# alibaba-mmai-research/CLIP-FSAR

Measured on AMD Instinct MI355X. Metric: episodes/sec (5-way 1-shot, 8 frames, ViT-B/16), higher is better.
Workload: dtype bf16; 1 GPU; BASELINE config[1]: 5-way 1-shot, 1 query/class, 8x224^2 frames, ViT-B/16, random-init CLIP weights, synthetic structured frames; frames_per_episode=80, precision=bf16, parallelism=episodes sharded over 1 rank(s); one all-gather of accuracies, launcher=single process

## Files before the change

clip-fsar_amd/build.py:

```python
from __future__ import annotations

import collections
import os
import subprocess
import sys

HERE = os.path.dirname(os.path.abspath(__file__))
CSRC = os.path.join(HERE, "csrc")
LIB = os.path.join(HERE, "libclipfsar_hip.so")
SOURCES = ["runtime.hip", "gemm.hip", "gemm_vit.hip", "frame_gemm.hip", "rowops.hip", "attention.hip", "tail.hip", "conv.hip"]
HIPCC = os.environ.get("HIPCC", "/opt/rocm/bin/hipcc")
DEV_LIB = os.path.join(HERE, "libclipfsar_hip_dev.so")
FLAGS = ["--offload-arch=gfx950", "-O3", "-std=c++17", "-fPIC", "-fvisibility=hidden", "-Wall", "-Wno-unused-function",
         "-Rpass-analysis=kernel-resource-usage"]
NO_PACKED_FP32 = ["-Xclang", "-target-feature", "-Xclang", "-packed-fp32-ops"]
SOURCE_FLAGS = {src: NO_PACKED_FP32 for src in SOURCES}
USAGE = os.path.join(HERE, "build", "resource_usage.json")
SideLib = collections.namedtuple("SideLib", "source lib usage")
SIDE_LIBS = {name: SideLib(name + ".hip", os.path.join(HERE, "libclipfsar_%s.so" % name),
                           os.path.join(HERE, "build", name, "resource_usage.json"))
             for name in ("gallery", "gallery_text", "stream", "pool", "ingest", "live")}


MORE_SIDE_LIBS = {name: SideLib(name + ".hip", os.path.join(HERE, "libclipfsar_%s.so" % name),
                                os.path.join(HERE, "build", name, "resource_usage.json"))
                  for name in ("groups",)}


def side_lib_names() -> list:
    return list(SIDE_LIBS)


def every_side_lib_names() -> list:
    return list(SIDE_LIBS) + list(MORE_SIDE_LIBS)


def _side_lib(name) -> SideLib:
    return SIDE_LIBS[name] if name in SIDE_LIBS else MORE_SIDE_LIBS[name]


def _parse_usage(text: str) -> dict:
    import re
    out, cur = {}, None
    for line in text.splitlines():
        m = re.search(r"remark: Function Name: (\S+)", line)
        if m:
            cur = out.setdefault(m.group(1), {})
            continue
        if cur is None:
            continue
        for key, pat in (("vgprs", r"remark:\s+VGPRs: (\d+)"), ("agprs", r"remark:\s+AGPRs: (\d+)"),
                         ("scratch", r"ScratchSize \[bytes/lane\]: (\d+)"), ("spills", r"VGPRs Spill: (\d+)"),
                         ("occupancy", r"Occupancy \[waves/SIMD\]: (\d+)")):
            m = re.search(pat, line)
            if m:
                cur[key] = int(m.group(1))
    return out


def _includes(path, seen=None) -> set:
    import re
    seen = set() if seen is None else seen
    path = os.path.normpath(path)
    if path not in seen:
        seen.add(path)
        for inc in re.findall(r'^#include "([^"]+)"', open(path).read(), flags=re.M):
            _includes(os.path.join(os.path.dirname(path), inc), seen)
    return seen


def _side_deps(name) -> list:
    return sorted(_includes(os.path.join(CSRC, _side_lib(name).source))) + [os.path.abspath(__file__)]


def _product_deps() -> list:
    ours = set().union(*(_includes(os.path.join(CSRC, s)) for s in SOURCES))
    side_only = set().union(*(_includes(os.path.join(CSRC, sl.source)) for sl in map(_side_lib, every_side_lib_names()))) - ours
    return [p for p in (os.path.join(CSRC, f) for f in sorted(os.listdir(CSRC))) if p not in side_only] + [
        os.path.join(os.path.dirname(HERE), "include", "clipfsar_hip.h"), os.path.abspath(__file__)]


def _stale(lib, deps) -> bool:
    if not os.path.exists(lib):
        return True
    t = os.path.getmtime(lib)
    return any(os.path.getmtime(d) > t for d in deps)


PACKED_LIB = os.path.join(HERE, "libclipfsar_hip_packed.so")


def _compile(src, obj, extra, verbose) -> dict:
    cmd = [HIPCC] + FLAGS + extra + ["-c", os.path.join(CSRC, src), "-o", obj]
    if verbose:
        print(" ".join(cmd), flush=True)
    p = subprocess.run(cmd, stdout=subprocess.PIPE, stderr=subprocess.STDOUT, text=True)
    if p.returncode != 0:
        raise RuntimeError("hipcc failed on %s:\n%s" % (src, p.stdout))
    rest = "\n".join(l for l in p.stdout.splitlines() if "-Rpass-analysis=kernel-resource-usage" not in l)
    if verbose and rest.strip():
        print(rest)
    return _parse_usage(p.stdout)


def _link(lib, objs, usage, usage_path, verbose) -> str:
    import json
    with open(usage_path, "w") as f:
        json.dump(usage, f, indent=0, sort_keys=True)
    cmd = [HIPCC, "--offload-arch=gfx950", "-shared", "-fPIC", "-o", lib] + objs
    if verbose:
        print(" ".join(cmd), flush=True)
    subprocess.check_call(cmd)
    return lib


def build_side(name, force: bool = False, verbose: bool = True) -> str:
    sl = _side_lib(name)
    if not force and not _stale(sl.lib, _side_deps(name)):
        return sl.lib
    bdir = os.path.dirname(sl.usage)
    os.makedirs(bdir, exist_ok=True)
    obj = os.path.join(bdir, sl.source.replace(".hip", ".o"))
    return _link(sl.lib, [obj], _compile(sl.source, obj, NO_PACKED_FP32, verbose), sl.usage, verbose)


def build(force: bool = False, verbose: bool = True, dev: bool = False, packed: bool = False, variant: str = "", defs=()) -> str:
    if not (dev or packed or variant):
        for name in every_side_lib_names():
            build_side(name, force=force, verbose=verbose)
    LIB_OUT = os.path.join(HERE, "libclipfsar_hip_%s.so" % variant) if variant else (PACKED_LIB if packed else (DEV_LIB if dev else LIB))
    if not force and not _stale(LIB_OUT, _product_deps()):
        return LIB_OUT
    bdir = os.path.join(HERE, "build", variant or "packed") if (packed or variant) else (os.path.join(HERE, "build", "dev") if dev else os.path.join(HERE, "build"))
    os.makedirs(bdir, exist_ok=True)
    extra = (os.environ.get("CFSAR_BUILD_DEFS", "").split() if dev else []) + list(defs)
    fenced = not (packed or "-DCFSAR_PACKED_FP32" in extra)
    extra = (["-DCFSAR_DEV"] if dev else []) + [e for e in extra if e != "-DCFSAR_PACKED_FP32"]
    objs = [os.path.join(bdir, src.replace(".hip", ".o")) for src in SOURCES]
    from concurrent.futures import ThreadPoolExecutor
    with ThreadPoolExecutor(len(SOURCES)) as pool:
        reports = list(pool.map(lambda so: _compile(so[0], so[1], extra + (SOURCE_FLAGS.get(so[0], []) if fenced else []), verbose),
                                zip(SOURCES, objs)))
    usage = {}
    for r in reports:
        usage.update(r)
    return _link(LIB_OUT, objs, usage, USAGE if not (dev or packed or variant) else os.path.join(bdir, "resource_usage.json"), verbose)


if __name__ == "__main__":
    _v = sys.argv[sys.argv.index("--variant") + 1] if "--variant" in sys.argv else ""
    _d = [a for a in sys.argv[1:] if a.startswith("-D")]
    print(build(force="--force" in sys.argv, dev="--dev" in sys.argv, packed="--packed" in sys.argv, variant=_v, defs=_d))
```

clip-fsar_amd/engine.py:

```python
from __future__ import annotations

import math

import os

import torch

from . import hip


FP16_SPLIT_DEFAULT = ""
FP16_MCORR_DEFAULT = "qkv,out,fc,pr"
FP16_STRICT_SPLIT_DEFAULT = "qkv"
FP16_STRICT_MCORR_DEFAULT = "out,fc,pr"
FP16_STRICT_DEEP_LAYERS = 12
FP16_STRICT_SPLIT_DEEP_DEFAULT = "qkv,fc"
FP16_STRICT_MCORR_DEEP_DEFAULT = "out,pr"


def _round_up(x, m):
    return (x + m - 1) // m * m


class HipViT:

    OPTIONS = {"fp16_wide": True, "fp16_lo": True, "fp16_rawmeans": True, "fused_umeans": True, "fused_omeans": True, "fuse_stats": True,
               "fused_patch": True, "strict_front": True, "strict_o_pair": False}

    def __init__(self, arch: dict, sd: dict, prefix: str = "", precision: str = "bf16", device="cuda", stream_dtype=None, fp16_split=None, fp16_mcorr=None,
                 options=None):
        self.strict = precision == "fp16_strict"
        if self.strict:
            precision = "fp16"
        if precision not in ("bf16", "fp16", "fp32"):
            raise ValueError("precision must be 'bf16', 'fp16', 'fp16_strict' or 'fp32'")
        opt = dict(self.OPTIONS)
        for k, v in (options or {}).items():
            if k not in opt:
                raise ValueError("HipViT: unknown option %r (known: %s)" % (k, ", ".join(sorted(opt))))
            opt[k] = bool(v)
        self.arch = dict(arch)
        self.precision = precision
        self.dev = torch.device(device)
        self.cd = {"bf16": torch.bfloat16, "fp16": torch.float16, "fp32": torch.float32}[precision]
        if stream_dtype is None:
            stream_dtype = "fp32" if precision == "fp32" else "fp16"
        if stream_dtype not in ("fp16", "fp32") or (precision == "fp32" and stream_dtype != "fp32") or (precision == "fp16" and stream_dtype != "fp16"):
            raise ValueError("stream_dtype must be 'fp32' (bf16 / fp32 precision) or 'fp16' (bf16 / fp16 precision)")
        self.xd = torch.float16 if stream_dtype == "fp16" else torch.float32
        D, P = arch["width"], arch["patch"]
        if D != arch["heads"] * 64:
            raise ValueError("HipViT needs head_dim == 64 (width %d, heads %d)" % (D, arch["heads"]))
        self.D, self.P, self.L, self.H, self.E = D, P, arch["layers"], arch["heads"], arch["embed"]
        self.grid = arch["res"] // P
        self.ntok = self.grid * self.grid + 1
        kq = 32 if precision == "fp32" else 64
        self.kpad = _round_up(3 * P * P, kq)

        def g(name):
            t = sd[prefix + name]
            if not isinstance(t, torch.Tensor):
                t = torch.from_numpy(t)
            return t.detach().to(device=self.dev, dtype=torch.float32).contiguous()

        cd = self.cd
        wc = torch.zeros(D, self.kpad, device=self.dev, dtype=torch.float32)
        wc[:, :3 * P * P] = g("conv1.weight").reshape(D, -1)
        self.w_patch = wc.to(cd).contiguous()
        self.fused_patch = bool(opt["fused_patch"] and P in hip.PATCH_EMBED_SLOTS and cd in (torch.bfloat16, torch.float16)
                                and self.xd == torch.float16)
        if self.fused_patch:
            self.w_patch_fused = self.w_patch if P == 16 else hip.patch_embed_weight(g("conv1.weight"), P, cd)
        self.cls = g("class_embedding")
        self.pos = g("positional_embedding")
        self.ln_pre = (g("ln_pre.weight"), g("ln_pre.bias"))
        self.ln_post = (g("ln_post.weight"), g("ln_post.bias"))
        self.w_proj_t = g("proj").t().contiguous()
        self.blocks = []
        for i in range(self.L):
            b = "transformer.resblocks.%d." % i
            self.blocks.append(dict(
                ln1=(g(b + "ln_1.weight"), g(b + "ln_1.bias")),
                ln2=(g(b + "ln_2.weight"), g(b + "ln_2.bias")),
                w_qkv=g(b + "attn.in_proj_weight").to(cd).contiguous(), b_qkv=g(b + "attn.in_proj_bias"),
                w_out=g(b + "attn.out_proj.weight").to(cd).contiguous(), b_out=g(b + "attn.out_proj.bias"),
                w_fc=g(b + "mlp.c_fc.weight").to(cd).contiguous(), b_fc=g(b + "mlp.c_fc.bias"),
                w_pr=g(b + "mlp.c_proj.weight").to(cd).contiguous(), b_pr=g(b + "mlp.c_proj.bias")))
        self.fold = (precision in ("bf16", "fp16") and self.xd == torch.float16 and D % 64 == 0 and D >= 128
                     and (precision == "fp16" or os.environ.get("CFSAR_LN_FOLD", "1") != "0"))
        if precision == "fp16":
            if not self.fold:
                raise ValueError("precision 'fp16' needs the LayerNorm-folded block (width a multiple of 64, >= 128)")
            wmax16 = max(float(blk[k].float().abs().max()) for blk in self.blocks for k in ("w_out", "w_pr"))
            wmax16 = max(wmax16, float(self.w_patch.float().abs().max()))
            if not wmax16 < 6.0e4:
                raise ValueError("precision 'fp16': a weight exceeds the fp16 range (max |w| = %.3g); use 'bf16' or 'fp32'" % wmax16)
        self.wide = precision == "fp16" and opt["fp16_wide"]
        self.two_word = self.wide and opt["fp16_lo"]
        sp_default, mc_default = FP16_SPLIT_DEFAULT, FP16_MCORR_DEFAULT
        if self.strict:
            deep = self.L > FP16_STRICT_DEEP_LAYERS
            sp_default = FP16_STRICT_SPLIT_DEEP_DEFAULT if deep else FP16_STRICT_SPLIT_DEFAULT
            mc_default = FP16_STRICT_MCORR_DEEP_DEFAULT if deep else FP16_STRICT_MCORR_DEFAULT
        sp = os.environ.get("CFSAR_FP16_SPLIT", sp_default if fp16_split is None else fp16_split) if precision == "fp16" else ""
        self.split = set(t for t in sp.split(",") if t)
        mc = os.environ.get("CFSAR_FP16_MCORR", mc_default if fp16_mcorr is None else fp16_mcorr) if precision == "fp16" else ""
        self.mcorr = set(t for t in mc.split(",") if t)
        if not (self.split | self.mcorr) <= {"qkv", "out", "fc", "pr"}:
            raise ValueError("CFSAR_FP16_SPLIT / CFSAR_FP16_MCORR: names out of qkv,out,fc,pr expected, got %r / %r" % (sp, mc))
        self.mcorr -= self.split
        if self.mcorr and self.ntok < 128:
            self.split |= self.mcorr
            self.mcorr = set()
        if not self.wide and precision == "fp16" and (self.mcorr or self.split & {"out", "pr"}):
            import warnings
            warnings.warn("HipViT: option fp16_wide=False drops the per-frame correction / split residual weights (%s / %s)" % (
                ",".join(sorted(self.mcorr)) or "-", ",".join(sorted(self.split & {"out", "pr"})) or "-"))
            self.mcorr = set()
            self.split -= {"out", "pr"}

        def hilo(W32):
            hi = W32.to(torch.float16)
            lo = (W32 - hi.float()).to(torch.float16)
            return torch.cat([hi, lo], 1).contiguous()

        def lo_word(W32):
            return (W32 - W32.to(torch.float16).float()).to(torch.bfloat16).contiguous()

        last = len(self.blocks) - 1
        for i, blk in enumerate(self.blocks if (self.split or self.mcorr) else []):
            b = "transformer.resblocks.%d." % i
            for key, name in (("out", "attn.out_proj.weight"), ("pr", "mlp.c_proj.weight")):
                if key in self.split:
                    blk["w_" + key] = hilo(g(b + name))
                elif key in self.mcorr:
                    blk["wlo_" + key] = lo_word(g(b + name))
                    if i == last:
                        blk["ws_" + key] = hilo(g(b + name))
        if self.fold:
            for i, blk in enumerate(self.blocks):
                b = "transformer.resblocks.%d." % i
                for tag, wname, bname, ln in (("qkv", "attn.in_proj_weight", "attn.in_proj_bias", "ln1"),
                                              ("fc", "mlp.c_fc.weight", "mlp.c_fc.bias", "ln2")):
                    W = g(b + wname)
                    gamma, beta = blk[ln]
                    if tag in self.split:
                        Wg = hilo(W * gamma[None, :])
                    else:
                        Wg = (W * gamma[None, :]).to(torch.float16).contiguous()
                    if tag in self.mcorr:
                        blk["wlo_" + tag] = lo_word(W * gamma[None, :])
                        if i == len(self.blocks) - 1:
                            Ws = hilo(W * gamma[None, :]) if tag == "fc" else hilo((W * gamma[None, :])[:D])
                            blk["wgs_" + tag] = Ws
                            blk["cs_" + tag] = Ws.double().sum(1).float().contiguous()
                    blk["wg_" + tag] = Wg
                    blk["c_" + tag] = Wg.double().sum(1).float().contiguous()
                    blk["cx_" + tag] = (W * gamma[None, :]).double().sum(1).float().contiguous()
                    blk["d_" + tag] = (W.double() @ beta.double() + g(b + bname).double()).float().contiguous()
            big = max(float(max(blk[k].abs().max() for k in ("c_qkv", "d_qkv", "c_fc", "d_fc"))) for blk in self.blocks)
            wmax = max(float(max(blk[k].float().abs().max() for k in ("wg_qkv", "wg_fc"))) for blk in self.blocks)
            if not (big < 3.0e4 and wmax < 6.0e4):
                import warnings
                if precision == "fp16":
                    raise ValueError("precision 'fp16': folded weights / vectors exceed the fp16 range (max |c|,|d| = %.3g, "
                                     "max |W gamma| = %.3g); use 'bf16' or 'fp32'" % (big, wmax))
                warnings.warn("LayerNorm folding disabled: folded weights / vectors exceed the fp16 range (max |c|,|d| = %.3g, "
                              "max |W gamma| = %.3g); using the unfolded block" % (big, wmax))
                self.fold = False
            if self.fold:
                for blk in self.blocks:
                    blk["w_qkv"] = blk["w_fc"] = None
        self.prune_last = os.environ.get("CFSAR_FULL_LAST_BLOCK", "0") != "1"
        self.fuse_stats = bool(self.fold) and hip.lnfold_partials_ok(self.D, self.D // 64) and opt["fuse_stats"]
        self.fused_umeans = opt["fused_umeans"]
        self.fused_omeans = opt["fused_omeans"]
        self.rawmeans = (opt["fp16_rawmeans"] and self.fused_umeans and self.fused_omeans
                         and all(k in self.mcorr for k in ("out", "pr")) and all(k in self.mcorr | self.split for k in ("qkv", "fc"))
                         and bool(self.mcorr & {"qkv", "fc"}))
        if self.rawmeans:
            for i, blk in enumerate(self.blocks):
                bb = "transformer.resblocks.%d." % i
                blk["wb_out"] = g(bb + "attn.out_proj.weight").to(torch.bfloat16).contiguous()
                blk["wb_pr"] = g(bb + "mlp.c_proj.weight").to(torch.bfloat16).contiguous()
        if self.mcorr & {"qkv", "fc"}:
            self.fuse_stats = False
        self.strict_front = self.o_pair = False
        if self.strict:
            if not (self.two_word and self.fold and D % 4 == 0 and D <= 1024):
                raise ValueError("precision 'fp16_strict' needs the two-word stream (options fp16_wide / fp16_lo) and a width <= 1024")
            self.strict_front = bool(opt["strict_front"])
            if self.strict_front:
                self.fused_patch = False
                w32 = wc
                w_hi = w32.to(torch.float16)
                w_lo = (w32 - w_hi.float()).to(torch.float16)
                self.w_patch3 = torch.cat([w_hi, w_hi, w_lo], 1).contiguous()
            self.o_pair = bool(opt["strict_o_pair"]) and self.fused_omeans and "out" in self.mcorr and D % 128 == 0
            if self.o_pair:
                for i, blk in enumerate(self.blocks):
                    W = g("transformer.resblocks.%d.attn.out_proj.weight" % i)
                    Wh = W.to(torch.float16)
                    blk["w3_out"] = torch.cat([Wh, Wh, (W - Wh.float()).to(torch.float16)], 1).contiguous()
        self._slots = {}
        self.max_frames_32bit = (2 ** 32 - 1) // (self.ntok * 4 * self.D * 2) - 1
        if self.strict_front:
            self.max_frames_32bit = min(self.max_frames_32bit, (2 ** 32 - 1) // ((self.ntok - 1) * 3 * self.kpad * 2) - 1)

    def _workspace(self, F_, slot=0):
        cap, ws = self._slots.get(slot, (0, None))
        if F_ > cap:
            M, D, cd, dev = F_ * self.ntok, self.D, self.cd, self.dev
            ws = dict(
                x=torch.empty(M, D, device=dev, dtype=self.xd),
                h=torch.empty(M, D, device=dev, dtype=cd),
                qkv=torch.empty(M, 3 * D, device=dev, dtype=cd),
                o=torch.empty(M, 2 * D if self.o_pair else D, device=dev, dtype=cd),
                u=torch.empty(M, 4 * D, device=dev, dtype=cd),
                c=torch.empty(F_, D, device=dev, dtype=torch.float32))
            if self.strict_front:
                ws["patches"] = torch.empty(F_ * (self.ntok - 1), 3 * self.kpad, device=dev, dtype=cd)
                ws["tok32"] = torch.empty(F_ * (self.ntok - 1), D, device=dev, dtype=torch.float32)
            elif not self.fused_patch:
                ws["patches"] = torch.empty(F_ * (self.ntok - 1), self.kpad, device=dev, dtype=cd)
            if self.fold:
                ws["part"] = torch.empty(M, D // 64, 2, device=dev, dtype=torch.float32)
                ws["rstat"] = torch.empty(M, 4, device=dev, dtype=torch.float32)
            if self.mcorr:
                ws["colsum"] = torch.empty((M // 96 + 2) * 2 * 4 * D, device=dev, dtype=torch.int32)
                ws["mU"] = torch.empty(F_ * 4 * D, device=dev, dtype=torch.bfloat16)
                ws["mX"] = torch.empty(F_, D, device=dev, dtype=torch.bfloat16)
                ws["xbar"] = torch.empty(F_, D, device=dev, dtype=torch.bfloat16)
                ws["mA"] = torch.empty(F_ * 4 * D, device=dev, dtype=torch.bfloat16)
                ws["corr"] = torch.empty(F_ * 4 * D, device=dev, dtype=torch.float32)
            if self.two_word:
                ws["xlo"] = torch.empty(M, D, device=dev, dtype=torch.float16)
                ws["xlc"] = torch.empty(F_, D, device=dev, dtype=torch.float16)
                ws["c32"] = torch.empty(F_, D, device=dev, dtype=torch.float32)
            ws["xc"] = torch.empty(F_, D, device=dev, dtype=self.xd)
            ws["hc"] = torch.empty(F_, D, device=dev, dtype=cd)
            ws["oc"] = torch.empty(F_, D, device=dev, dtype=cd)
            ws["uc"] = torch.empty(F_, 4 * D, device=dev, dtype=cd)
            ws["partc"] = torch.empty(F_, D // 64 if D % 64 == 0 else 1, 2, device=dev, dtype=torch.float32)
            ws["rstatc"] = torch.empty(F_, 4, device=dev, dtype=torch.float32)
            self._slots[slot] = (F_, ws)
        return ws

    def forward(self, frame_sets, feats_out=None, row_maps=None, taps=None, slot=0):
        if isinstance(frame_sets, torch.Tensor):
            frame_sets = [frame_sets]
        counts = [int(f.shape[0]) for f in frame_sets]
        F_ = sum(counts)
        if row_maps is None:
            row_maps, off = [], 0
            for c in counts:
                row_maps.append((0, 0, off))
                off += c
        if feats_out is None:
            feats_out = torch.empty(F_, self.E, device=self.dev, dtype=torch.float32)
        ws = self._workspace(F_, slot)
        N, D, npatch = self.ntok, self.D, self.ntok - 1
        M = F_ * N
        x, h, qkv, o, u = ws["x"], ws["h"], ws["qkv"], ws["o"], ws["u"]
        off = 0
        for fr, c in zip(frame_sets, counts):
            if fr.shape[1:] != (3, self.arch["res"], self.arch["res"]):
                raise RuntimeError("frames must be [F,3,%d,%d], got %s" % (self.arch["res"], self.arch["res"], tuple(fr.shape)))
            if self.fused_patch:
                hip.patch_embed(fr, self.w_patch_fused, self.pos, self.cls, x[off * N:(off + c) * N], self.P)
            elif self.strict_front:
                hip.im2col_patches_split(fr, ws["patches"][off * npatch:(off + c) * npatch], self.P)
            else:
                hip.im2col_patches(fr, ws["patches"][off * npatch:(off + c) * npatch], self.P)
            off += c
        if self.strict_front:
            hip.gemm(ws["patches"], self.w_patch3, ws["tok32"], M=F_ * npatch, N=D, K=3 * self.kpad, ldo=D)
            hip.embed_finish_pair(ws["tok32"], self.cls, self.pos, self.ln_pre[0], self.ln_pre[1], x, ws["xlo"], F_, N, D)
        else:
            if not self.fused_patch:
                hip.gemm(ws["patches"], self.w_patch, x, residual=self.pos, M=F_ * npatch, N=D, K=self.kpad, ldo=D, ldr=D,
                         row_group=npatch, row_gap=1, row_off=1, res_mod=npatch, res_off=1)
                hip.cls_rows(x, self.cls, self.pos, F_, N, D)
            hip.layernorm(x, x, self.ln_pre[0], self.ln_pre[1], M, D)
        if taps is not None:
            taps["ln_pre"] = (x[:M].float() + ws["xlo"][:M].float()) if self.strict_front else x[:M].clone()
        xc_final = None
        es = x.element_size()

        def class_rows(src, dst, row_elems, elem_bytes):
            hip.copy_rows_strided(src, N * row_elems * elem_bytes, dst, row_elems * elem_bytes, F_, row_elems * elem_bytes)

        if self.fold:
            part, rstat, S = ws["part"], ws["rstat"], D // 64
            xlo = ws["xlo"] if self.two_word else None
            if xlo is not None and not self.strict_front:
                xlo[:M].zero_()
            hip.row_stats(x, rstat, M, D)
            prune = self.prune_last and taps is None
            fuse = self.fuse_stats
            in_part = False
            split = self.split

            mcorr = self.mcorr
            raw = self.rawmeans and bool(mcorr)
            xbar = ws["xbar"][:F_] if raw else None
            if raw:
                hip.frame_col_means(x, xbar, F_, N)

            def mc(blk, key, A, rs=None, wrows=None, means=None):
                if key not in mcorr:
                    return None
                wlo = blk["wlo_" + key] if wrows is None else blk["wlo_" + key][wrows]
                Kd, Nn = A.shape[1], wlo.shape[0]
                if raw and key in ("qkv", "fc"):
                    mA = xbar
                elif means is not None:
                    mA = means
                else:
                    mA = ws["mA"][:F_ * Kd].view(F_, Kd)
                    hip.frame_col_means(A, mA, F_, N, rowstats=rs)
                cr = ws["corr"][:F_ * Nn].view(F_, Nn)
                hip.corr_gemm(mA, wlo, cr)
                return cr

            def fold(xx, wg, out, c, d, pt, rs, act=hip.ACT_NONE, rows=M, from_part=False, sp=False, corr=None, umeans=None, corr_raw=False):
                if sp or corr is not None or umeans is not None:
                    hip.gemm_lnfold_hp(xx, wg, out, c, d, rowstats=None if from_part else rs, partial=pt if from_part else None,
                                       slots=S if from_part else 0, rowstats_ws=rs, act=act, M=rows, wsplit=sp, corr=corr,
                                       corr_tokens=N if (corr is not None or umeans is not None) else 0, colmean_out=umeans,
                                       colsum_ws=ws["colsum"] if umeans is not None else None, corr_raw=corr_raw and corr is not None)
                elif from_part:
                    hip.gemm_lnfold_partials(xx, wg, out, c, d, pt, S, rs, act=act, M=rows)
                else:
                    hip.gemm_lnfold(xx, wg, out, c, d, rs, act=act, M=rows)

            def resid(A, blk, key, xx, xl, pt, rows, corr=None, cls=False):
                if self.o_pair and key == "out" and not cls:
                    hip.gemm_residual_wide(A, blk["w3_out"], xx, xl, blk["b_out"], pt, M=rows, wsplit=2)
                elif self.wide and cls and key in mcorr:
                    hip.gemm_residual_wide(A, blk["ws_" + key], xx, xl, blk["b_" + key], pt, M=rows, wsplit=True)
                elif self.wide:
                    hip.gemm_residual_wide(A, blk["w_" + key], xx, xl, blk["b_" + key], pt, M=rows, wsplit=key in split, corr=corr,
                                           corr_tokens=N if corr is not None else 0)
                else:
                    hip.gemm_residual_stats(A, blk["w_" + key], xx, blk["b_" + key], pt, M=rows)

            for i, b in enumerate(self.blocks):
                if prune and i == self.L - 1:
                    xc, oc, uc, partc, rstatc = ws["xc"][:F_], ws["oc"][:F_], ws["uc"][:F_], ws["partc"][:F_], ws["rstatc"][:F_]
                    xlc = ws["xlc"][:F_] if xlo is not None else None
                    kv = qkv.view(-1)[:M * 2 * D].view(M, 2 * D)
                    fold(x, b["wg_qkv"][D:], kv, b["cx_qkv" if raw else "c_qkv"][D:], b["d_qkv"][D:], part, rstat, from_part=in_part, sp="qkv" in split,
                         corr=mc(b, "qkv", x, rstat, wrows=slice(D, 3 * D)), corr_raw=raw)
                    class_rows(x, xc, D, es)
                    if xlo is not None:
                        class_rows(xlo, xlc, D, 2)
                    if in_part:
                        class_rows(part, partc, 2 * S, 4)
                    else:
                        class_rows(rstat, rstatc, 4, 4)
                    qc = ws["hc"][:F_]
                    if "qkv" in mcorr:
                        fold(xc, b["wgs_qkv"], qc, b["cs_qkv"], b["d_qkv"][:D], partc, rstatc, rows=F_, from_part=in_part, sp=True)
                    else:
                        fold(xc, b["wg_qkv"][:D], qc, b["c_qkv"][:D], b["d_qkv"][:D], partc, rstatc, rows=F_, from_part=in_part, sp="qkv" in split)
                    hip.vit_attention_cls(None, oc, F_, N, D, self.H, q=qc, kv=kv)
                    resid(oc, b, "out", xc, xlc, partc, F_, cls=True)
                    if not fuse:
                        hip.ln_stats_finalize(partc, rstatc, F_, S, D)
                    if "fc" in mcorr:
                        fold(xc, b["wgs_fc"], uc, b["cs_fc"], b["d_fc"], partc, rstatc, act=hip.ACT_QUICKGELU, rows=F_, from_part=fuse, sp=True)
                    else:
                        fold(xc, b["wg_fc"], uc, b["c_fc"], b["d_fc"], partc, rstatc, act=hip.ACT_QUICKGELU, rows=F_, from_part=fuse, sp="fc" in split)
                    resid(uc, b, "pr", xc, xlc, None, F_, cls=True)
                    xc_final = xc
                    break
                fold(x, b["wg_qkv"], qkv, b["cx_qkv" if raw else "c_qkv"], b["d_qkv"], part, rstat, from_part=in_part, sp="qkv" in split,
                     corr=mc(b, "qkv", x, rstat), corr_raw=raw)
                if self.o_pair:
                    mO = ws["mX"][:F_]
                    hip.vit_attention_pair(qkv, o, mO, F_, N, D, self.H)
                elif "out" in mcorr and self.fused_omeans:
                    mO = ws["mX"][:F_]
                    hip.vit_attention_means(qkv, o, mO, F_, N, D, self.H)
                else:
                    mO = None
                    hip.vit_attention(qkv, o, F_, N, D, self.H)
                resid(o, b, "out", x, xlo, part, M, corr=None if self.o_pair else mc(b, "out", o, means=mO))
                if raw:
                    hip.mean_update_gemm(mO, b["wb_out"], b["b_out"], xbar)
                if not fuse:
                    hip.ln_stats_finalize(part, rstat, M, S, D)
                um = ws["mU"][:F_ * 4 * D].view(F_, 4 * D) if ("pr" in mcorr and self.fused_umeans) else None
                fold(x, b["wg_fc"], u, b["cx_fc" if raw else "c_fc"], b["d_fc"], part, rstat, act=hip.ACT_QUICKGELU, from_part=fuse, sp="fc" in split,
                     corr=mc(b, "fc", x, rstat), umeans=um, corr_raw=raw)
                resid(u, b, "pr", x, xlo, part, M, corr=mc(b, "pr", u, means=um))
                if raw:
                    hip.mean_update_gemm(um, b["wb_pr"], b["b_pr"], xbar)
                if fuse:
                    in_part = True
                else:
                    hip.ln_stats_finalize(part, rstat, M, S, D)
                if taps is not None:
                    taps["block%d" % i] = (x[:M].float() + xlo[:M].float()) if xlo is not None else x[:M].clone()
        for i, b in enumerate(self.blocks if not self.fold else []):
            if self.prune_last and taps is None and i == self.L - 1:
                xc, hc, oc, uc = ws["xc"][:F_], ws["hc"][:F_], ws["oc"][:F_], ws["uc"][:F_]
                hip.layernorm(x, h, b["ln1"][0], b["ln1"][1], M, D)
                hip.gemm(h, b["w_qkv"], qkv, bias=b["b_qkv"], M=M)
                hip.vit_attention_cls(qkv, oc, F_, N, D, self.H)
                class_rows(x, xc, D, es)
                hip.gemm(oc, b["w_out"], xc, bias=b["b_out"], residual=xc, M=F_)
                hip.layernorm(xc, hc, b["ln2"][0], b["ln2"][1], F_, D)
                hip.gemm(hc, b["w_fc"], uc, bias=b["b_fc"], act=hip.ACT_QUICKGELU, M=F_)
                hip.gemm(uc, b["w_pr"], xc, bias=b["b_pr"], residual=xc, M=F_)
                xc_final = xc
                break
            hip.layernorm(x, h, b["ln1"][0], b["ln1"][1], M, D)
            hip.gemm(h, b["w_qkv"], qkv, bias=b["b_qkv"], M=M)
            hip.vit_attention(qkv, o, F_, N, D, self.H)
            hip.gemm(o, b["w_out"], x, bias=b["b_out"], residual=x, M=M)
            hip.layernorm(x, h, b["ln2"][0], b["ln2"][1], M, D)
            hip.gemm(h, b["w_fc"], u, bias=b["b_fc"], act=hip.ACT_QUICKGELU, M=M)
            hip.gemm(u, b["w_pr"], x, bias=b["b_pr"], residual=x, M=M)
            if taps is not None:
                taps["block%d" % i] = x[:M].clone()
        if self.fold and self.two_word:
            if xc_final is None:
                xc_final = ws["xc"][:F_]
                class_rows(x, xc_final, D, es)
                class_rows(ws["xlo"], ws["xlc"][:F_], D, 2)
            hip.f16_pair_to_f32(xc_final, ws["xlc"][:F_], ws["c32"][:F_])
            hip.layernorm(ws["c32"], ws["c"], self.ln_post[0], self.ln_post[1], F_, D, in_stride=D, out_stride=D)
        elif xc_final is not None:
            hip.layernorm(xc_final, ws["c"], self.ln_post[0], self.ln_post[1], F_, D, in_stride=D, out_stride=D)
        else:
            hip.layernorm(x, ws["c"], self.ln_post[0], self.ln_post[1], F_, D, in_stride=N * D, out_stride=D)
        off = 0
        for c, (rg, gap, roff) in zip(counts, row_maps):
            hip.gemm(ws["c"][off:off + c], self.w_proj_t, feats_out, M=c, N=self.E, K=D, ldo=self.E,
                     row_group=rg, row_gap=gap, row_off=roff)
            off += c
        return feats_out


class HipResNet:

    IMPLICIT_MIN_TILES = 128

    def __init__(self, arch: dict, sd: dict, prefix: str = "", precision: str = "bf16", device="cuda"):
        if precision == "fp16_strict":
            raise ValueError("precision 'fp16_strict' exists for the ViT towers; the RN50 tower's mode for the 1e-3 contract is 'fp32'")
        if precision not in ("bf16", "fp16", "fp32"):
            raise ValueError("precision must be 'bf16', 'fp16' or 'fp32'")
        self.arch = dict(arch)
        self.dev = torch.device(device)
        self.cd = {"bf16": torch.bfloat16, "fp16": torch.float16, "fp32": torch.float32}[precision]
        self.kq = 32 if precision == "fp32" else 64
        self.E = arch["embed"]
        self.width, self.layers, self.heads = arch["width"], arch["layers"], arch["heads"]
        self.max_frames_32bit = (2 ** 32 - 1) // ((arch["res"] // 2) ** 2 * self.width * (4 if precision == "fp32" else 2)) - 1
        if (self.width * 32) % self.heads or (self.width * 32) // self.heads > 128:
            raise ValueError("attention-pool head_dim must be <= 128")

        def g(name):
            t = sd[prefix + name]
            if not isinstance(t, torch.Tensor):
                t = torch.from_numpy(t)
            return t.detach().to(device=self.dev, dtype=torch.float32)

        def fold(conv, bn):
            w = g(conv + ".weight")
            s_ = g(bn + ".weight") / torch.sqrt(g(bn + ".running_var") + 1e-5)
            b = g(bn + ".bias") - g(bn + ".running_mean") * s_
            w = w * s_.reshape(-1, 1, 1, 1)
            cout, cin, k, _ = w.shape
            w2 = w.permute(0, 2, 3, 1).reshape(cout, k * k * cin)
            kpad = _round_up(w2.shape[1], self.kq)
            wp = torch.zeros(cout, kpad, device=self.dev, dtype=torch.float32)
            wp[:, :w2.shape[1]] = w2
            if self.cd == torch.float16 and float(wp.abs().max()) > 6.0e4:
                raise ValueError("precision 'fp16': the BatchNorm-folded weights of %s leave the fp16 range (max |w| = %.3g); use 'bf16' or "
                                 "'fp32'" % (conv, float(wp.abs().max())))
            return wp.to(self.cd).contiguous(), b.contiguous()

        self.stem = [fold("conv1", "bn1"), fold("conv2", "bn2"), fold("conv3", "bn3")]
        self.stem_direct = None
        if self.cd != torch.float32 and (self.width // 2) in (8, 16, 32, 64):
            s1 = g("bn1.weight") / torch.sqrt(g("bn1.running_var") + 1e-5)
            self.stem_direct = ((g("conv1.weight") * s1.reshape(-1, 1, 1, 1)).contiguous(),
                                (g("bn1.bias") - g("bn1.running_mean") * s1).contiguous())
        self.blocks = []
        inplanes = self.width
        for li, (planes, nb) in enumerate(zip((self.width, self.width * 2, self.width * 4, self.width * 8), self.layers), 1):
            for bi in range(nb):
                stride = 2 if (li > 1 and bi == 0) else 1
                b = "layer%d.%d." % (li, bi)
                blk = dict(stride=stride, planes=planes, inplanes=inplanes, c1=fold(b + "conv1", b + "bn1"),
                           c2=fold(b + "conv2", b + "bn2"), c3=fold(b + "conv3", b + "bn3"), down=None)
                if stride > 1 or inplanes != planes * 4:
                    blk["down"] = fold(b + "downsample.0", b + "downsample.1")
                self.blocks.append(blk)
                inplanes = planes * 4
        self.C = inplanes
        self.pos = g("attnpool.positional_embedding").contiguous()
        self.w_q = g("attnpool.q_proj.weight").to(self.cd).contiguous()
        self.b_q = g("attnpool.q_proj.bias").contiguous()
        self.w_kv = torch.cat([g("attnpool.k_proj.weight"), g("attnpool.v_proj.weight")], 0).to(self.cd).contiguous()
        self.b_kv = torch.cat([g("attnpool.k_proj.bias"), g("attnpool.v_proj.bias")], 0).contiguous()
        self.w_c = g("attnpool.c_proj.weight").contiguous()
        self.b_c = g("attnpool.c_proj.bias").contiguous()

    def _conv3x3(self, x, F_, H, W, C, wb, stride):
        w, b = wb
        if (stride == 1 and self.cd != torch.float32 and C >= 8 and (C & (C - 1)) == 0
                and ((F_ * H * W + 255) // 256) * ((w.shape[0] + 255) // 256) >= self.IMPLICIT_MIN_TILES):
            out = torch.empty(F_ * H * W, w.shape[0], device=self.dev, dtype=self.cd)
            hip.conv3x3(x, w, out, F_, H, W, C, bias=b, relu=True)
            return out, H, W
# ... 218 lines not shown
```

Baseline: 362.7 episodes/s.

## Fold key/value projections into last-block class-token attention

In the pruned last block, the full K/V projection GEMM over all tokens is no longer computed. Each frame's class query is folded through the key weights into a per-head vector g. Attention then scores against the LayerNorm-normalised hidden states directly, using an online softmax. The weighted token sum is projected through the value weights afterwards. This replaces an M x 2D x D GEMM with small per-frame matvecs, at the cost of a new custom kernel, an extra fp32 buffer, and fp16 precision risk in the folded path.

Measured after the change: 367.1 episodes/s (median of 6 runs). 1.2% higher.

```diff
diff --git a/clip-fsar_amd/build.py b/clip-fsar_amd/build.py
--- a/clip-fsar_amd/build.py
+++ b/clip-fsar_amd/build.py
@@ -27,6 +27,11 @@
                   for name in ("groups",)}
 
 
+TOWER_LIBS = {name: SideLib(name + ".hip", os.path.join(HERE, "libclipfsar_%s.so" % name),
+                            os.path.join(HERE, "build", name, "resource_usage.json"))
+              for name in ("lastblock",)}
+
+
 def side_lib_names() -> list:
     return list(SIDE_LIBS)
 
@@ -35,8 +40,19 @@
     return list(SIDE_LIBS) + list(MORE_SIDE_LIBS)
 
 
+def tower_lib_names() -> list:
+    return list(TOWER_LIBS)
+
+
+def _all_lib_names() -> list:
+    return every_side_lib_names() + tower_lib_names()
+
+
 def _side_lib(name) -> SideLib:
-    return SIDE_LIBS[name] if name in SIDE_LIBS else MORE_SIDE_LIBS[name]
+    for libs in (SIDE_LIBS, MORE_SIDE_LIBS):
+        if name in libs:
+            return libs[name]
+    return TOWER_LIBS[name]
 
 
 def _parse_usage(text: str) -> dict:
@@ -75,7 +91,7 @@
 
 def _product_deps() -> list:
     ours = set().union(*(_includes(os.path.join(CSRC, s)) for s in SOURCES))
-    side_only = set().union(*(_includes(os.path.join(CSRC, sl.source)) for sl in map(_side_lib, every_side_lib_names()))) - ours
+    side_only = set().union(*(_includes(os.path.join(CSRC, sl.source)) for sl in map(_side_lib, _all_lib_names()))) - ours
     return [p for p in (os.path.join(CSRC, f) for f in sorted(os.listdir(CSRC))) if p not in side_only] + [
         os.path.join(os.path.dirname(HERE), "include", "clipfsar_hip.h"), os.path.abspath(__file__)]
 
@@ -126,7 +142,7 @@
 
 def build(force: bool = False, verbose: bool = True, dev: bool = False, packed: bool = False, variant: str = "", defs=()) -> str:
     if not (dev or packed or variant):
-        for name in every_side_lib_names():
+        for name in _all_lib_names():
             build_side(name, force=force, verbose=verbose)
     LIB_OUT = os.path.join(HERE, "libclipfsar_hip_%s.so" % variant) if variant else (PACKED_LIB if packed else (DEV_LIB if dev else LIB))
     if not force and not _stale(LIB_OUT, _product_deps()):
diff --git a/clip-fsar_amd/csrc/lastblock.hip b/clip-fsar_amd/csrc/lastblock.hip
--- /dev/null
+++ b/clip-fsar_amd/csrc/lastblock.hip
@@ -0,0 +1,341 @@
+#include "side_lib.h"
+#include "../../include/clipfsar_lastblock.h"
+
+namespace {
+
+constexpr int CHUNK = CFLB_TOKEN_CHUNK, FB = CFLB_FRAME_BATCH;
+static_assert(CHUNK == 32 && FB == 16, "one MFMA K step of tokens, one MFMA tile of frames");
+typedef __fp16 tr_f16x4 __attribute__((__vector_size__(4 * sizeof(__fp16))));
+
+__device__ __forceinline__ f16x4 lds_read_tr(const unsigned char* p) {
+    return __builtin_bit_cast(f16x4, __builtin_amdgcn_ds_read_tr16_b64_v4f16((__attribute__((address_space(3))) tr_f16x4*)(p)));
+}
+
+__device__ __forceinline__ f32x4 mfma16(f16x8 a, f16x8 b, f32x4 c) { return __builtin_amdgcn_mfma_f32_16x16x32_f16(a, b, c, 0, 0, 0); }
+
+__device__ __forceinline__ float row16_sum(float v) {
+    v = cfsar_dpp_sum8(v);
+    return v + cfsar_dpp_move<0x140>(v);
+}
+
+template <typename TQ>
+__global__ __launch_bounds__(256) void key_fold_kernel(const TQ* __restrict__ q, const _Float16* __restrict__ wk_t, _Float16* __restrict__ g,
+                                                       float* __restrict__ G, int F, int D, int heads) {
+    __shared__ float Gp[4][FB];
+    const int lane = threadIdx.x & 63, w = threadIdx.x >> 6, c = lane & 15, kg = lane >> 4;
+    const int f0 = blockIdx.x * FB, h = blockIdx.y;
+    f16x8 a[2];
+#pragma unroll
+    for (int ks = 0; ks < 2; ++ks) {
+#pragma unroll
+        for (int e = 0; e < 8; ++e) a[ks][e] = (_Float16)0.f;
+        if (f0 + c < F) {
+            const TQ* qp = q + (size_t)(f0 + c) * D + h * 64 + ks * 32 + 8 * kg;
+#pragma unroll
+            for (int e = 0; e < 8; ++e) a[ks][e] = (_Float16)(float)qp[e];
+        }
+    }
+    float gsum[4] = {0.f, 0.f, 0.f, 0.f};
+    for (int nt = w; nt < D / 16; nt += 4) {
+        const int k = nt * 16 + c;
+        const _Float16* wp = wk_t + ((size_t)h * D + k) * 64 + 8 * kg;
+        f32x4 acc = {0.f, 0.f, 0.f, 0.f};
+        acc = mfma16(a[0], *reinterpret_cast<const f16x8*>(wp), acc);
+        acc = mfma16(a[1], *reinterpret_cast<const f16x8*>(wp + 32), acc);
+#pragma unroll
+        for (int r = 0; r < 4; ++r) {
+            const _Float16 gv = (_Float16)(acc[r] * 0.125f);
+            gsum[r] += (float)gv;
+            const int fr = f0 + 4 * kg + r;
+            if (fr < F) g[((size_t)fr * heads + h) * D + k] = gv;
+        }
+    }
+#pragma unroll
+    for (int r = 0; r < 4; ++r) {
+        const float s = row16_sum(gsum[r]);
+        if (c == 0) Gp[w][4 * kg + r] = s;
+    }
+    __syncthreads();
+    if (threadIdx.x < FB && f0 + (int)threadIdx.x < F) {
+        const int i = threadIdx.x;
+        G[(size_t)(f0 + i) * heads + h] = ((Gp[0][i] + Gp[1][i]) + Gp[2][i]) + Gp[3][i];
+    }
+}
+
+template <typename TO>
+__global__ __launch_bounds__(256) void value_fold_kernel(const float* __restrict__ z, const _Float16* __restrict__ wv,
+                                                         const float* __restrict__ d_v, TO* __restrict__ oc, int F, int D, int heads) {
+    const int lane = threadIdx.x & 63, w = threadIdx.x >> 6, c = lane & 15, kg = lane >> 4;
+    const int f0 = blockIdx.x * FB, h = blockIdx.y, n = h * 64 + w * 16 + c;
+    const bool rowok = f0 + c < F;
+    const float* zp = z + ((size_t)(rowok ? f0 + c : f0) * heads + h) * D + 8 * kg;
+    const _Float16* wp = wv + (size_t)n * D + 8 * kg;
+    f32x4 acc = {0.f, 0.f, 0.f, 0.f};
+    for (int k = 0; k < D; k += 32) {
+        const f32x4 z0 = *reinterpret_cast<const f32x4*>(zp + k), z1 = *reinterpret_cast<const f32x4*>(zp + k + 4);
+        f16x8 hi, lo;
+#pragma unroll
+        for (int e = 0; e < 8; ++e) {
+            const float v = rowok ? (e < 4 ? z0[e] : z1[e - 4]) : 0.f;
+            hi[e] = (_Float16)v;
+            lo[e] = (_Float16)(v - (float)hi[e]);
+        }
+        const f16x8 b = *reinterpret_cast<const f16x8*>(wp + k);
+        acc = mfma16(lo, b, acc);
+        acc = mfma16(hi, b, acc);
+    }
+    const float bias = d_v[n];
+#pragma unroll
+    for (int r = 0; r < 4; ++r) {
+        const int fr = f0 + 4 * kg + r;
+        if (fr < F) oc[(size_t)fr * D + n] = (TO)(acc[r] + bias);
+    }
+}
+
+template <int NT>
+__global__ __launch_bounds__(256, NT <= 12 ? 2 : 1) void class_attend_kernel(const _Float16* __restrict__ x, const _Float16* __restrict__ g,
+                                                           const float* __restrict__ G, const float* __restrict__ partial, int slots,
+                                                           const float* __restrict__ rowstats, float eps, float* __restrict__ z,
+                                                           int ntok, int D, int heads) {
+    extern __shared__ __attribute__((aligned(16))) unsigned char smem[];
+    const int tid = threadIdx.x, lane = tid & 63, w = tid >> 6, c = lane & 15, kg = lane >> 4;
+    const int f = blockIdx.x, stride = 2 * D + 32;
+    unsigned char* xs = smem;
+    float* Sp = reinterpret_cast<float*>(smem + CHUNK * stride);
+    f16x8* afrag = reinterpret_cast<f16x8*>(Sp + 4 * CHUNK * 16);
+    float* mu_s = reinterpret_cast<float*>(afrag + 64);
+    float *sd_s = mu_s + CHUNK, *rsd_s = sd_s + CHUNK, *alpha_s = rsd_s + CHUNK;
+    float* fin_s = alpha_s + 16;
+    const size_t row0 = (size_t)f * ntok;
+
+    f16x8 gfrag[(NT + 1) / 2];
+#pragma unroll
+    for (int i = 0; i < (NT + 1) / 2; ++i) {
+#pragma unroll
+        for (int e = 0; e < 8; ++e) gfrag[i][e] = (_Float16)0.f;
+        const int ks = w + 4 * i;
+        if (ks < 2 * heads && c < heads) gfrag[i] = *reinterpret_cast<const f16x8*>(g + ((size_t)f * heads + c) * D + ks * 32 + 8 * kg);
+    }
+    const float Gh = c < heads ? G[(size_t)f * heads + c] : 0.f;
+    f32x4 acc[NT];
+#pragma unroll
+    for (int i = 0; i < NT; ++i) acc[i] = f32x4{0.f, 0.f, 0.f, 0.f};
+    float m_run = -INFINITY, l_run = 0.f, c_run = 0.f;
+    const int pieces = D / 8;
+
+    uint4 v[NT];
+    float4 st;
+    const int srow = tid >> 3, sq = tid & 7;
+    const float invD = 1.0f / (float)D;
+    auto fetch = [&](int t0) {
+#pragma unroll
+        for (int i = 0; i < NT; ++i) {
+            v[i] = make_uint4(0u, 0u, 0u, 0u);
+            if (i < heads) {
+                const int idx = tid + 256 * i, r = idx / pieces, p = idx - r * pieces;
+                if (t0 + r < ntok) v[i] = *reinterpret_cast<const uint4*>(x + (row0 + t0 + r) * D + p * 8);
+            }
+        }
+        st = make_float4(0.f, 0.f, 0.f, 0.f);
+        if (t0 + srow < ntok) {
+            const size_t m = row0 + t0 + srow;
+            if (rowstats) {
+                if (sq == 0) st = *reinterpret_cast<const float4*>(rowstats + m * 4);
+            } else {
+                const float2* pp = reinterpret_cast<const float2*>(partial) + m * slots + 2 * sq;
+                if (2 * sq < slots) st.x = pp[0].x, st.y = pp[0].y;
+                if (2 * sq + 1 < slots) st.z = pp[1].x, st.w = pp[1].y;
+            }
+        }
+    };
+    fetch(0);
+
+    for (int t0 = 0; t0 < ntok; t0 += CHUNK) {
+#pragma unroll
+        for (int i = 0; i < NT; ++i) {
+            if (i < heads) {
+                const int idx = tid + 256 * i, r = idx / pieces, p = idx - r * pieces;
+                *reinterpret_cast<uint4*>(xs + r * stride + p * 16) = v[i];
+            }
+        }
+        {
+            float mean = st.x, sd = st.y, rsd = st.z;
+            if (!rowstats) {
+                const float s = cfsar_dpp_sum8(st.x + st.z), ss = cfsar_dpp_sum8(st.y + st.w);
+                mean = s * invD;
+                sd = sqrtf(fmaxf(ss * invD - mean * mean, 0.f) + eps);
+                rsd = 1.0f / sd;
+            }
+            if (t0 + srow >= ntok) mean = 0.f, sd = 1.f, rsd = 0.f;
+            if (sq == 0) mu_s[srow] = mean, sd_s[srow] = sd, rsd_s[srow] = rsd;
+        }
+        __syncthreads();
+        if (t0 + CHUNK < ntok) fetch(t0 + CHUNK);
+        {
+            f32x4 s0 = {0.f, 0.f, 0.f, 0.f}, s1 = {0.f, 0.f, 0.f, 0.f};
+#pragma unroll
+            for (int i = 0; i < (NT + 1) / 2; ++i) {
+                const int ks = w + 4 * i;
+                if (ks < 2 * heads) {
+                    const unsigned char* ap = xs + c * stride + (ks * 32 + 8 * kg) * 2;
+                    s0 = mfma16(*reinterpret_cast<const f16x8*>(ap), gfrag[i], s0);
+                    s1 = mfma16(*reinterpret_cast<const f16x8*>(ap + 16 * stride), gfrag[i], s1);
+                }
+            }
+#pragma unroll
+            for (int r = 0; r < 4; ++r) {
+                Sp[(w * CHUNK + 4 * kg + r) * 16 + c] = s0[r];
+                Sp[(w * CHUNK + 16 + 4 * kg + r) * 16 + c] = s1[r];
+            }
+        }
+        __syncthreads();
+        if (w == 0) {
+            float s[8], cm = -INFINITY;
+#pragma unroll
+            for (int j = 0; j < 8; ++j) {
+                const int t = 8 * kg + j;
+                const float S = ((Sp[t * 16 + c] + Sp[(CHUNK + t) * 16 + c]) + Sp[(2 * CHUNK + t) * 16 + c]) + Sp[(3 * CHUNK + t) * 16 + c];
+                s[j] = t0 + t < ntok ? (S - mu_s[t] * Gh) * rsd_s[t] : -INFINITY;
+                cm = fmaxf(cm, s[j]);
+            }
+            cm = fmaxf(cm, __shfl_xor(cm, 16, 64));
+            cm = fmaxf(cm, __shfl_xor(cm, 32, 64));
+            const float m_new = fmaxf(m_run, cm);
+            const float alpha = expf(m_run - m_new);
+            float ls = 0.f, cs = 0.f;
+            f16x8 wv;
+#pragma unroll
+            for (int j = 0; j < 8; ++j) {
+                const int t = 8 * kg + j;
+                wv[j] = (_Float16)(expf(s[j] - m_new) * rsd_s[t]);
+                const float wf = (float)wv[j];
+                ls = fmaf(wf, sd_s[t], ls);
+                cs = fmaf(wf, mu_s[t], cs);
+            }
+            ls += __shfl_xor(ls, 16, 64);
+            ls += __shfl_xor(ls, 32, 64);
+            cs += __shfl_xor(cs, 16, 64);
+            cs += __shfl_xor(cs, 32, 64);
+            l_run = fmaf(l_run, alpha, ls);
+            c_run = fmaf(c_run, alpha, cs);
+            m_run = m_new;
+            afrag[lane] = wv;
+            if (kg == 0) alpha_s[c] = alpha;
+        }
+        __syncthreads();
+        {
+            const f16x8 a = afrag[lane];
+            float al[4];
+#pragma unroll
+            for (int r = 0; r < 4; ++r) al[r] = alpha_s[4 * kg + r];
+            const unsigned char* bp = xs + (8 * kg + (c >> 2)) * stride + (4 * (c & 3)) * 2;
+#pragma unroll
+            for (int i = 0; i < NT; ++i) {
+                if (i < heads) {
+                    const unsigned char* p = bp + (i * 4 + w) * 32;
+                    const f16x4 b0 = lds_read_tr(p), b1 = lds_read_tr(p + 4 * stride);
+                    const f16x8 b = {b0[0], b0[1], b0[2], b0[3], b1[0], b1[1], b1[2], b1[3]};
+#pragma unroll
+                    for (int r = 0; r < 4; ++r) acc[i][r] *= al[r];
+                    acc[i] = mfma16(a, b, acc[i]);
+                }
+            }
+        }
+        __syncthreads();
+    }
+    if (w == 0 && kg == 0) fin_s[c] = c_run, fin_s[16 + c] = 1.0f / l_run;
+    __syncthreads();
+#pragma unroll
+    for (int i = 0; i < NT; ++i) {
+        if (i < heads) {
+            const int col = (i * 4 + w) * 16 + c;
+#pragma unroll
+            for (int r = 0; r < 4; ++r) {
+                const int h = 4 * kg + r;
+                if (h < heads) z[((size_t)f * heads + h) * D + col] = (acc[i][r] - fin_s[h]) * fin_s[16 + h];
+            }
+        }
+    }
+}
+
+bool aligned16(const void* p) { return ((uintptr_t)p & 15u) == 0; }
+
+int check_dims(const char* who, int F, int D, int heads) {
+    SIDE_REQUIRE(heads >= 1 && heads <= CFLB_MAX_HEADS && D == 64 * heads && F >= 1,
+                 "%s: bad shape (F=%d D=%d heads=%d; F >= 1, 1 <= heads <= %d, D == 64 * heads)", who, F, D, heads, CFLB_MAX_HEADS);
+    return 0;
+}
+
+int attend_lds_bytes(int D) { return CHUNK * (2 * D + 32) + 4 * CHUNK * 16 * 4 + 64 * 16 + (3 * CHUNK + 16 + 32) * 4; }
+
+template <int NT>
+int launch_attend(const char* who, const void* x, const void* g, const float* G, const float* partial, int slots, const float* rowstats,
+                  float eps, float* z, int F, int ntok, int D, int heads, hipStream_t s) {
+    const int lds = attend_lds_bytes(D);
+    if (lds > 48 * 1024) {
+        const hipError_t e = hipFuncSetAttribute(reinterpret_cast<const void*>(class_attend_kernel<NT>),
+                                                 hipFuncAttributeMaxDynamicSharedMemorySize, lds);
+        if (e != hipSuccess) return fail("%s: %d bytes of LDS: %s", who, lds, hipGetErrorString(e));
+    }
+    hipLaunchKernelGGL(class_attend_kernel<NT>, dim3((unsigned)F), dim3(256), lds, s, static_cast<const _Float16*>(x),
+                       static_cast<const _Float16*>(g), G, partial, slots, rowstats, eps, z, ntok, D, heads);
+    return check_launch(who);
+}
+
+}
+
+extern "C" int cflb_version(void) { return 100;  }
+extern "C" int cflb_abi_version(void) { return CFLB_ABI_VERSION; }
+extern "C" const char* cflb_last_error(void) { return g_err; }
+
+extern "C" int cflb_key_fold(const void* q, int dtype, const void* wk_t, void* g, float* G, int F, int D, int heads, cflb_stream_t stream) {
+    const char* who = "cflb_key_fold";
+    SIDE_REQUIRE(q && wk_t && g && G, "%s: null pointer", who);
+    if (check_dims(who, F, D, heads)) return 1;
+    SIDE_REQUIRE(dtype == CFLB_BF16 || dtype == CFLB_F16, "%s: bad dtype %d", who, dtype);
+    SIDE_REQUIRE(aligned16(q) && aligned16(wk_t) && aligned16(g), "%s: q, wk_t and g must be 16-byte aligned", who);
+    const dim3 grid((unsigned)((F + FB - 1) / FB), (unsigned)heads);
+    hipStream_t s = static_cast<hipStream_t>(stream);
+    if (dtype == CFLB_BF16)
+        hipLaunchKernelGGL(key_fold_kernel<__bf16>, grid, dim3(256), 0, s, static_cast<const __bf16*>(q), static_cast<const _Float16*>(wk_t),
+                           static_cast<_Float16*>(g), G, F, D, heads);
+    else
+        hipLaunchKernelGGL(key_fold_kernel<_Float16>, grid, dim3(256), 0, s, static_cast<const _Float16*>(q),
+                           static_cast<const _Float16*>(wk_t), static_cast<_Float16*>(g), G, F, D, heads);
+    return check_launch(who);
+}
+
+extern "C" int cflb_class_attend(const void* x, const void* g, const float* G, const float* partial, int slots, const float* rowstats,
+                                 float eps, float* z, int F, int ntok, int D, int heads, cflb_stream_t stream) {
+    const char* who = "cflb_class_attend";
+    SIDE_REQUIRE(x && g && G && z, "%s: null pointer", who);
+    if (check_dims(who, F, D, heads)) return 1;
+    SIDE_REQUIRE(ntok >= 1 && (long long)F * ntok <= 0x7fffffffLL, "%s: bad shape (ntok=%d F=%d; ntok >= 1, F * ntok below 2^31)", who, ntok, F);
+    SIDE_REQUIRE((partial != nullptr) != (rowstats != nullptr), "%s: exactly one of partial and rowstats is needed", who);
+    SIDE_REQUIRE(partial ? (slots >= 1 && slots <= 16) : slots == 0, "%s: slots=%d (1 .. 16 with partial, 0 with rowstats)", who, slots);
+    SIDE_REQUIRE(eps > 0.f, "%s: eps must be > 0", who);
+    SIDE_REQUIRE(aligned16(x) && aligned16(g) && aligned16(z) && aligned16(partial) && aligned16(rowstats),
+                 "%s: x, g, z and the statistics must be 16-byte aligned", who);
+    hipStream_t s = static_cast<hipStream_t>(stream);
+    if (heads <= 2) return launch_attend<2>(who, x, g, G, partial, slots, rowstats, eps, z, F, ntok, D, heads, s);
+    if (heads <= 12) return launch_attend<12>(who, x, g, G, partial, slots, rowstats, eps, z, F, ntok, D, heads, s);
+    return launch_attend<16>(who, x, g, G, partial, slots, rowstats, eps, z, F, ntok, D, heads, s);
+}
+
+extern "C" int cflb_value_fold(const float* z, const void* wv, const float* d_v, void* oc, int dtype, int F, int D, int heads,
+                               cflb_stream_t stream) {
+    const char* who = "cflb_value_fold";
+    SIDE_REQUIRE(z && wv && d_v && oc, "%s: null pointer", who);
+    if (check_dims(who, F, D, heads)) return 1;
+    SIDE_REQUIRE(dtype == CFLB_BF16 || dtype == CFLB_F16, "%s: bad dtype %d", who, dtype);
+    SIDE_REQUIRE(aligned16(z) && aligned16(wv), "%s: z and wv must be 16-byte aligned", who);
+    const dim3 grid((unsigned)((F + FB - 1) / FB), (unsigned)heads);
+    hipStream_t s = static_cast<hipStream_t>(stream);
+    if (dtype == CFLB_BF16)
+        hipLaunchKernelGGL(value_fold_kernel<__bf16>, grid, dim3(256), 0, s, z, static_cast<const _Float16*>(wv), d_v,
+                           static_cast<__bf16*>(oc), F, D, heads);
+    else
+        hipLaunchKernelGGL(value_fold_kernel<_Float16>, grid, dim3(256), 0, s, z, static_cast<const _Float16*>(wv), d_v,
+                           static_cast<_Float16*>(oc), F, D, heads);
+    return check_launch(who);
+}
diff --git a/clip-fsar_amd/engine.py b/clip-fsar_amd/engine.py
--- a/clip-fsar_amd/engine.py
+++ b/clip-fsar_amd/engine.py
@@ -25,7 +25,7 @@
 class HipViT:
 
     OPTIONS = {"fp16_wide": True, "fp16_lo": True, "fp16_rawmeans": True, "fused_umeans": True, "fused_omeans": True, "fuse_stats": True,
-               "fused_patch": True, "strict_front": True, "strict_o_pair": False}
+               "fused_patch": True, "strict_front": True, "strict_o_pair": False, "fold_last_kv": True}
 
     def __init__(self, arch: dict, sd: dict, prefix: str = "", precision: str = "bf16", device="cuda", stream_dtype=None, fp16_split=None, fp16_mcorr=None,
                  options=None):
@@ -172,6 +172,10 @@
                 for blk in self.blocks:
                     blk["w_qkv"] = blk["w_fc"] = None
         self.prune_last = os.environ.get("CFSAR_FULL_LAST_BLOCK", "0") != "1"
+        self.fold_last_kv = bool(opt["fold_last_kv"] and precision == "bf16" and self.fold and self.H <= 16)
+        if self.fold_last_kv:
+            blk = self.blocks[-1]
+            blk["wk_t"] = blk["wg_qkv"][D:2 * D].view(self.H, 64, D).transpose(1, 2).contiguous()
         self.fuse_stats = bool(self.fold) and hip.lnfold_partials_ok(self.D, self.D // 64) and opt["fuse_stats"]
         self.fused_umeans = opt["fused_umeans"]
         self.fused_omeans = opt["fused_omeans"]
@@ -237,6 +241,10 @@
                 ws["xlo"] = torch.empty(M, D, device=dev, dtype=torch.float16)
                 ws["xlc"] = torch.empty(F_, D, device=dev, dtype=torch.float16)
                 ws["c32"] = torch.empty(F_, D, device=dev, dtype=torch.float32)
+            if self.fold_last_kv:
+                ws["g"] = torch.empty(F_, self.H, D, device=dev, dtype=torch.float16)
+                ws["G"] = torch.empty(F_, self.H, device=dev, dtype=torch.float32)
+                ws["z"] = torch.empty(F_, self.H, D, device=dev, dtype=torch.float32)
             ws["xc"] = torch.empty(F_, D, device=dev, dtype=self.xd)
             ws["hc"] = torch.empty(F_, D, device=dev, dtype=cd)
             ws["oc"] = torch.empty(F_, D, device=dev, dtype=cd)
@@ -350,8 +358,9 @@
                     xc, oc, uc, partc, rstatc = ws["xc"][:F_], ws["oc"][:F_], ws["uc"][:F_], ws["partc"][:F_], ws["rstatc"][:F_]
                     xlc = ws["xlc"][:F_] if xlo is not None else None
                     kv = qkv.view(-1)[:M * 2 * D].view(M, 2 * D)
-                    fold(x, b["wg_qkv"][D:], kv, b["cx_qkv" if raw else "c_qkv"][D:], b["d_qkv"][D:], part, rstat, from_part=in_part, sp="qkv" in split,
-                         corr=mc(b, "qkv", x, rstat, wrows=slice(D, 3 * D)), corr_raw=raw)
+                    if not self.fold_last_kv:
+                        fold(x, b["wg_qkv"][D:], kv, b["cx_qkv" if raw else "c_qkv"][D:], b["d_qkv"][D:], part, rstat, from_part=in_part,
+                             sp="qkv" in split, corr=mc(b, "qkv", x, rstat, wrows=slice(D, 3 * D)), corr_raw=raw)
                     class_rows(x, xc, D, es)
                     if xlo is not None:
                         class_rows(xlo, xlc, D, 2)
@@ -364,7 +373,14 @@
                         fold(xc, b["wgs_qkv"], qc, b["cs_qkv"], b["d_qkv"][:D], partc, rstatc, rows=F_, from_part=in_part, sp=True)
                     else:
                         fold(xc, b["wg_qkv"][:D], qc, b["c_qkv"][:D], b["d_qkv"][:D], partc, rstatc, rows=F_, from_part=in_part, sp="qkv" in split)
-                    hip.vit_attention_cls(None, oc, F_, N, D, self.H, q=qc, kv=kv)
+                    if self.fold_last_kv:
+                        from . import lastblock_hip as lb
+                        g_, G_, z_ = ws["g"][:F_], ws["G"][:F_], ws["z"][:F_]
+                        lb.key_fold(qc, b["wk_t"], g_, G_)
+                        lb.class_attend(x, g_, G_, z_, N, partial=part if in_part else None, rowstats=None if in_part else rstat)
+                        lb.value_fold(z_, b["wg_qkv"][2 * D:], b["d_qkv"][2 * D:], oc)
+                    else:
+                        hip.vit_attention_cls(None, oc, F_, N, D, self.H, q=qc, kv=kv)
                     resid(oc, b, "out", xc, xlc, partc, F_, cls=True)
                     if not fuse:
                         hip.ln_stats_finalize(partc, rstatc, F_, S, D)
diff --git a/clip-fsar_amd/lastblock_hip.py b/clip-fsar_amd/lastblock_hip.py
--- /dev/null
+++ b/clip-fsar_amd/lastblock_hip.py
@@ -0,0 +1,91 @@
+from __future__ import annotations
+
+import os
+
+import torch
+
+import ctypes
+
+from . import _cabi, hip
+
+ABI_VERSION = 1
+LIB_PATH = os.path.join(os.path.dirname(os.path.abspath(__file__)), "libclipfsar_lastblock.so")
+MAX_HEADS = 16
+FRAME_BATCH = 16
+TOKEN_CHUNK = 32
+BF16, F16 = 1, 2
+_lib = None
+
+_c_int, _c_p, _c_f = ctypes.c_int, ctypes.c_void_p, ctypes.c_float
+
+SIGNATURES = {
+    "cflb_version": [],
+    "cflb_abi_version": [],
+    "cflb_key_fold": [_c_p, _c_int, _c_p, _c_p, _c_p, _c_int, _c_int, _c_int, _c_p],
+    "cflb_class_attend": [_c_p, _c_p, _c_p, _c_p, _c_int, _c_p, _c_f, _c_p, _c_int, _c_int, _c_int, _c_int, _c_p],
+    "cflb_value_fold": [_c_p, _c_p, _c_p, _c_p, _c_int, _c_int, _c_int, _c_int, _c_p],
+}
+
+
+def lib():
+    global _lib
+    if _lib is None:
+        _lib = _cabi.load(LIB_PATH, SIGNATURES, "cflb_", ABI_VERSION, "the folded last-block attention")
+    return _lib
+
+
+_check = _cabi.checker(lib, "cflb_")
+_shape = _cabi.shape_checker("lastblock_hip")
+_dev, _stream = hip._dev, hip._stream
+
+
+def _code(dtype):
+    if dtype == torch.bfloat16:
+        return BF16
+    if dtype == torch.float16:
+        return F16
+    raise RuntimeError("clip_fsar_amd.lastblock_hip: q / oc must be bf16 or fp16, got %s" % dtype)
+
+
+def key_weight(wk, heads):
+    D = wk.shape[1]
+    _shape(wk, (64 * heads, D), "wk")
+    return wk.view(heads, 64, D).transpose(1, 2).contiguous()
+
+
+def key_fold(q, wk_t, g, G):
+    F_, D = q.shape
+    heads = wk_t.shape[0]
+    _shape(wk_t, (heads, D, 64), "wk_t")
+    _shape(g, (F_, heads, D), "g")
+    _shape(G, (F_, heads), "G")
+    _check(lib().cflb_key_fold(_dev(q, None, "q"), _code(q.dtype), _dev(wk_t, torch.float16, "wk_t"), _dev(g, torch.float16, "g"),
+                               _dev(G, torch.float32, "G"), F_, D, heads, _stream()), "cflb_key_fold")
+
+
+def class_attend(x, g, G, z, ntok, partial=None, rowstats=None, eps=1e-5):
+    F_, heads, D = g.shape
+    M = F_ * ntok
+    if x.dim() != 2 or x.shape[1] != D or x.shape[0] < M:
+        raise RuntimeError("clip_fsar_amd.lastblock_hip: x has shape %s, expected [>= %d, %d]" % (tuple(x.shape), M, D))
+    _shape(G, (F_, heads), "G")
+    _shape(z, (F_, heads, D), "z")
+    slots = 0
+    if partial is not None:
+        if partial.dim() != 3 or partial.shape[0] < M or partial.shape[2] != 2:
+            raise RuntimeError("clip_fsar_amd.lastblock_hip: partial has shape %s, expected [>= %d, slots, 2]" % (tuple(partial.shape), M))
+        slots = partial.shape[1]
+    if rowstats is not None and (rowstats.dim() != 2 or rowstats.shape[0] < M or rowstats.shape[1] != 4):
+        raise RuntimeError("clip_fsar_amd.lastblock_hip: rowstats has shape %s, expected [>= %d, 4]" % (tuple(rowstats.shape), M))
+    _check(lib().cflb_class_attend(_dev(x, torch.float16, "x"), _dev(g, torch.float16, "g"), _dev(G, torch.float32, "G"),
+                                   hip._opt(partial, torch.float32, "partial"), slots, hip._opt(rowstats, torch.float32, "rowstats"),
+                                   float(eps), _dev(z, torch.float32, "z"), F_, int(ntok), D, heads, _stream()), "cflb_class_attend")
+
+
+def value_fold(z, wv, d_v, oc):
+    F_, heads, D = z.shape
+    _shape(wv, (D, D), "wv")
+    _shape(d_v, (D,), "d_v")
+    _shape(oc, (F_, D), "oc")
+    _check(lib().cflb_value_fold(_dev(z, torch.float32, "z"), _dev(wv, torch.float16, "wv"), _dev(d_v, torch.float32, "d_v"),
+                                 _dev(oc, None, "oc"), _code(oc.dtype), F_, D, heads, _stream()), "cflb_value_fold")
diff --git a/include/clipfsar_lastblock.h b/include/clipfsar_lastblock.h
--- /dev/null
+++ b/include/clipfsar_lastblock.h
@@ -0,0 +1,38 @@
+#ifndef CLIPFSAR_LASTBLOCK_H
+#define CLIPFSAR_LASTBLOCK_H
+
+#include <stdint.h>
+
+#ifdef __cplusplus
+extern "C" {
+#endif
+#if defined(__GNUC__) || defined(__clang__)
+#pragma GCC visibility push(default)
+#endif
+
+typedef void* cflb_stream_t;
+
+#define CFLB_ABI_VERSION 1
+#define CFLB_MAX_HEADS 16
+#define CFLB_FRAME_BATCH 16
+#define CFLB_TOKEN_CHUNK 32
+#define CFLB_BF16 1
+#define CFLB_F16 2
+int cflb_version(void);
+int cflb_abi_version(void);
+const char* cflb_last_error(void);
+
+int cflb_key_fold(const void* q, int dtype, const void* wk_t, void* g, float* G, int F, int D, int heads, cflb_stream_t stream);
+
+int cflb_class_attend(const void* x, const void* g, const float* G, const float* partial, int slots, const float* rowstats, float eps,
+                      float* z, int F, int ntok, int D, int heads, cflb_stream_t stream);
+
+int cflb_value_fold(const float* z, const void* wv, const float* d_v, void* oc, int dtype, int F, int D, int heads, cflb_stream_t stream);
+
+#if defined(__GNUC__) || defined(__clang__)
+#pragma GCC visibility pop
+#endif
+#ifdef __cplusplus
+}
+#endif
+#endif
```
